# kubeflow/Code-Intelligence

Hardware: AMD Instinct MI355X
Metric: LM tokens/sec (whole node) (higher is better)
Workload: dtype bf16; 1 GPU; model=AWD-LSTM 4x2400 emb800 vocab60000, global_batch=512, seq_len=512, parallelism=dp1, device=MI355X

## Files before the change

### code_intelligence_amd/ops/crossentropy.py

```python
from __future__ import annotations

import os

import torch
from torch import Tensor

from . import extension as ext

__all__ = ["tied_decoder_ce", "TiedDecoderCE"]

_EMPTY = {}


def _empty_f32(device) -> Tensor:
    key = str(device)
    if key not in _EMPTY:
        _EMPTY[key] = torch.empty(0, dtype=torch.float32, device=device)
    return _EMPTY[key]


def _fp8r_enabled() -> bool:
    return os.environ.get("CI_CE_FP8R", "1") == "1"


_STORE = 448.0

_ONEPASS_MAX_V = 256 * 32 * 8

_ce_side = None


def _ce_side_stream():
    global _ce_side
    if _ce_side is None:
        _ce_side = torch.cuda.Stream()
    return _ce_side


def _ce_overlap_enabled() -> bool:
    return os.environ.get("CI_CE_2STREAM", "0") == "1"


class _FusedCEFp8Function(torch.autograd.Function):

    @staticmethod
    def forward(ctx, h: Tensor, weight: Tensor, bias: Tensor, targets: Tensor):
        lib = ext.require()
        f8 = torch.float8_e4m3fn
        N, H = h.shape
        V = weight.shape[0]
        C = int(os.environ.get("CI_CE_CHUNK", _FusedCEFunction.CHUNK))
        dev = h.device
        lse = torch.empty(N, dtype=torch.float32, device=dev)
        tgt_logit = torch.empty(N, dtype=torch.float32, device=dev)
        b32 = bias.to(torch.float32) if bias is not None else _empty_f32(dev)
        tgt64 = targets.to(torch.int64)
        sa = (h.detach().abs().amax().float() / 448.0).clamp_min(1e-12)
        sw = (weight.detach().abs().amax().float() / 448.0).clamp_min(1e-12)
        h8 = torch.empty(h.shape, dtype=f8, device=dev)
        lib.quantize_e4m3(h.detach().contiguous(), h8, sa)
        w8 = torch.empty(weight.shape, dtype=f8, device=dev)
        lib.quantize_e4m3(weight.detach().contiguous(), w8, sw)
        w8_t = w8.t()
        w_t = weight.t()
        logits_full = None
        if os.environ.get("CI_CE_SAVE_LOGITS", "1") != "0":
            try:
                logits_full = torch.empty(N, V, dtype=h.dtype, device=dev)
            except torch.cuda.OutOfMemoryError:
                pass
        dlog8_full = None
        if logits_full is not None and V <= _ONEPASS_MAX_V \
                and H % 16 == 0 and V % 16 == 0 \
                and N % 16 == 0 and min(C, N) % 16 == 0:
            try:
                dlog8_full = torch.empty(N, V, dtype=f8, device=dev)
            except torch.cuda.OutOfMemoryError:
                pass
        onepass = dlog8_full is not None
        if onepass:
            inv_n = (torch.ones((), dtype=torch.float32, device=dev)
                     / N).reshape(1)
        scratch = None if logits_full is not None else \
            torch.empty(min(C, N), V, dtype=h.dtype, device=dev)
        for s in range(0, N, C):
            e = min(N, s + C)
            logits = logits_full[s:e] if logits_full is not None \
                else scratch[: e - s]
            if (e - s) % 16 == 0 and H % 16 == 0 and V % 16 == 0:
                torch._scaled_mm(h8[s:e], w8_t, scale_a=sa, scale_b=sw,
                                 out_dtype=h.dtype, out=logits)
            else:
                torch.mm(h[s:e], w_t, out=logits)
            if onepass:
                lib.ce_onepass_dual(logits, tgt64[s:e], b32, lse[s:e],
                                    inv_n, dlog8_full[s:e], _STORE)
            else:
                lib.ce_rowstats(logits, tgt64[s:e], b32, lse[s:e],
                                tgt_logit[s:e])
        wrows = weight.detach()[tgt64]
        tgt_logit = (h.detach() * wrows).sum(dim=1, dtype=torch.float32)
        if bias is not None:
            tgt_logit = tgt_logit + b32[tgt64]
        loss = (lse - tgt_logit).mean()
        ctx.save_for_backward(h, weight, b32, tgt64, lse, w8, sw)
        ctx.logits_full = logits_full
        ctx.dlog8_full = dlog8_full
        ctx.h8 = h8 if logits_full is None else None
        ctx.sa = sa
        ctx.chunk = C
        ctx.has_bias = bias is not None
        ctx.bias_dtype = bias.dtype if bias is not None else None
        return loss

    @staticmethod
    def backward(ctx, dloss: Tensor):
        lib = ext.require()
        f8 = torch.float8_e4m3fn
        h, weight, b32, targets, lse, w8, sw = ctx.saved_tensors
        logits_full = ctx.logits_full
        ctx.logits_full = None
        h8, sa = ctx.h8, ctx.sa
        ctx.h8 = None
        dlog8_full = ctx.dlog8_full
        ctx.dlog8_full = None
        onepass = dlog8_full is not None
        has_bias = ctx.has_bias
        N, H = h.shape
        V = weight.shape[0]
        C = ctx.chunk
        dev = h.device
        dh = torch.empty_like(h)
        scale = (dloss / N).to(torch.float32).reshape(1)
        sc_over_store = (scale.reshape(()) / _STORE)
        scratch8 = None if onepass else \
            torch.empty(min(C, N), V, dtype=f8, device=dev)
        Haug = H + 16 if has_bias else H
        h_aug = h
        if has_bias:
            h_aug = torch.zeros(N, Haug, dtype=h.dtype, device=dev)
            h_aug[:, :H] = h
            h_aug[:, H] = 1
        dw_aug = torch.zeros(V, Haug, dtype=torch.float32, device=dev)
        recompute = None if logits_full is not None else \
            torch.empty(min(C, N), V, dtype=h.dtype, device=dev)
        w8_cm = w8.t().contiguous().t()
        w8_t = w8.t()
        w_t = weight.t()
        bias_arg = b32 if has_bias else _empty_f32(dev)
        overlap = _ce_overlap_enabled() and logits_full is not None
        side = _ce_side_stream() if overlap else None
        main = torch.cuda.current_stream() if overlap else None
        for s in range(0, N, C):
            e = min(N, s + C)
            c = e - s
            fp8_chunk = c % 16 == 0 and H % 16 == 0 and V % 16 == 0
            if logits_full is not None:
                dlog = logits_full[s:e]
            else:
                dlog = recompute[:c]
                if fp8_chunk:
                    torch._scaled_mm(h8[s:e], w8_t, scale_a=sa, scale_b=sw,
                                     out_dtype=h.dtype, out=dlog)
                else:
                    torch.mm(h[s:e], w_t, out=dlog)
            if onepass:
                dlog8 = dlog8_full[s:e]
            else:
                lib.ce_dlogits_dual(dlog, targets[s:e], bias_arg, lse[s:e],
                                    scale, scratch8, _STORE)
                dlog8 = scratch8[:c]
            if fp8_chunk:
                torch._scaled_mm(dlog8, w8_cm, scale_a=sc_over_store,
                                 scale_b=sw, out_dtype=h.dtype, out=dh[s:e])
            else:
                torch.mm(dlog, weight, out=dh[s:e])
            if overlap:
                side.wait_stream(main)
                with torch.cuda.stream(side):
                    dw_aug += torch.mm(dlog.t(), h_aug[s:e])
            else:
                dw_aug += torch.mm(dlog.t(), h_aug[s:e])
        if overlap:
            main.wait_stream(side)
        dw = dw_aug[:, :H]
        db = dw_aug[:, H] if has_bias else None
        if onepass:
            dl = dloss.to(torch.float32)
            dw_out = torch.empty(V, H, dtype=weight.dtype, device=dev)
            torch.mul(dw, dl, out=dw_out)
            return (dh, dw_out,
                    (db * dl).to(ctx.bias_dtype) if has_bias else None, None)
        return (dh, dw.to(weight.dtype),
                db.to(ctx.bias_dtype) if has_bias else None, None)


class _FusedCEFunction(torch.autograd.Function):
    CHUNK = int(os.environ.get("CI_CE_CHUNK", "65536"))

    @staticmethod
    def forward(ctx, h: Tensor, weight: Tensor, bias: Tensor, targets: Tensor):
        lib = ext.require()
        N, H = h.shape
        V = weight.shape[0]
        C = int(os.environ.get("CI_CE_CHUNK", _FusedCEFunction.CHUNK))
        lse = torch.empty(N, dtype=torch.float32, device=h.device)
        tgt_logit = torch.empty(N, dtype=torch.float32, device=h.device)
        b32 = bias.to(torch.float32) if bias is not None else _empty_f32(h.device)
        tgt64 = targets.to(torch.int64)
        save_logits = os.environ.get("CI_CE_SAVE_LOGITS", "1") != "0"
        logits_full = None
        if save_logits:
            try:
                logits_full = torch.empty(N, V, dtype=h.dtype, device=h.device)
            except torch.cuda.OutOfMemoryError:
                logits_full = None
        scratch = None if logits_full is not None else \
            torch.empty(min(C, N), V, dtype=h.dtype, device=h.device)
        w_t = weight.t()
        for s in range(0, N, C):
            e = min(N, s + C)
            logits = logits_full[s:e] if logits_full is not None \
                else scratch[: e - s]
            torch.mm(h[s:e], w_t, out=logits)
            lib.ce_rowstats(logits, tgt64[s:e], b32, lse[s:e], tgt_logit[s:e])
        loss = (lse - tgt_logit).mean()
        ctx.save_for_backward(h, weight, b32, tgt64, lse)
        ctx.logits_full = logits_full
        ctx.chunk = C
        ctx.has_bias = bias is not None
        ctx.bias_dtype = bias.dtype if bias is not None else None
        return loss

    @staticmethod
    def backward(ctx, dloss: Tensor):
        lib = ext.require()
        h, weight, b32, targets, lse = ctx.saved_tensors
        logits_full = ctx.logits_full
        ctx.logits_full = None
        has_bias = ctx.has_bias
        N, H = h.shape
        V = weight.shape[0]
        C = ctx.chunk
        dh = torch.empty_like(h)
        scale = (dloss / N).to(torch.float32).reshape(1)
        scratch = None if logits_full is not None else \
            torch.empty(min(C, N), V, dtype=h.dtype, device=h.device)
        w_t = weight.t()
        bias_arg = b32 if has_bias else _empty_f32(h.device)
        Haug = H + 16 if has_bias else H
        h_aug = h
        if has_bias:
            h_aug = torch.zeros(N, Haug, dtype=h.dtype, device=h.device)
            h_aug[:, :H] = h
            h_aug[:, H] = 1
        dw_aug = torch.zeros(V, Haug, dtype=torch.float32, device=h.device)
        for s in range(0, N, C):
            e = min(N, s + C)
            if logits_full is not None:
                dlog = logits_full[s:e]
            else:
                dlog = scratch[: e - s]
                torch.mm(h[s:e], w_t, out=dlog)
            lib.ce_dlogits(dlog, targets[s:e], bias_arg, lse[s:e], scale)
            torch.mm(dlog, weight, out=dh[s:e])
            dw_aug += torch.mm(dlog.t(), h_aug[s:e])
        dw = dw_aug[:, :H]
        db = dw_aug[:, H] if has_bias else None
        return (dh, dw.to(weight.dtype),
                db.to(ctx.bias_dtype) if has_bias else None, None)


@torch.no_grad()
def tied_decoder_accuracy(h: Tensor, weight: Tensor, bias: Tensor | None,
                          targets: Tensor, chunk: int = 16384) -> Tensor:
    h2 = h.reshape(-1, h.shape[-1])
    t2 = targets.reshape(-1)
    w_t = weight.t()
    correct = torch.zeros((), dtype=torch.long, device=h.device)
    for s in range(0, h2.shape[0], chunk):
        e = min(h2.shape[0], s + chunk)
        logits = torch.mm(h2[s:e], w_t)
        if bias is not None:
            logits += bias
        correct += (logits.argmax(dim=1) == t2[s:e]).sum()
    return correct.float() / max(1, h2.shape[0])


def tied_decoder_ce(h: Tensor, weight: Tensor, bias: Tensor | None,
                    targets: Tensor) -> Tensor:
    if h.is_cuda:
        if _fp8r_enabled() and h.dtype == torch.bfloat16 \
                and torch.is_grad_enabled() and h.requires_grad:
            return _FusedCEFp8Function.apply(h, weight, bias, targets)
        return _FusedCEFunction.apply(h, weight, bias, targets)
    logits = torch.nn.functional.linear(h.float(), weight.float(),
                                        bias.float() if bias is not None else None)
    return torch.nn.functional.cross_entropy(logits, targets)


class TiedDecoderCE(torch.nn.Module):

    def __init__(self, decoder: torch.nn.Linear):
        super().__init__()
        self.decoder = decoder

    def forward(self, h: Tensor, targets: Tensor) -> Tensor:
        return tied_decoder_ce(h.reshape(-1, h.shape[-1]), self.decoder.weight,
                               self.decoder.bias, targets.reshape(-1))
```

### code_intelligence_amd/ops/csrc/bindings.cpp

```cpp
#include <torch/extension.h>
#include <string>
#include <vector>

namespace ci {
void lstm_seq_forward_lib(at::Tensor xp, at::Tensor bias, at::Tensor h0,
                          at::Tensor c0, at::Tensor w_hh, at::Tensor hs,
                          at::Tensor cs, at::Tensor gates);
void lstm_seq_forward_fused(at::Tensor xp, at::Tensor bias, at::Tensor h0,
                            at::Tensor c0, at::Tensor w_hh, at::Tensor hs,
                            at::Tensor cs, at::Tensor gates);
void lstm_seq_forward_lib_fp8(at::Tensor xp, at::Tensor bias, at::Tensor h0,
                              at::Tensor c0, at::Tensor w8, at::Tensor wscale,
                              at::Tensor hs, at::Tensor cs, at::Tensor gates);
void quantize_e4m3(at::Tensor src, at::Tensor dst, at::Tensor scale);
void lstm_seq_forward_gemv(at::Tensor xp, at::Tensor bias, at::Tensor h0,
                           at::Tensor c0, at::Tensor w_hh, at::Tensor hs,
                           at::Tensor cs, at::Tensor gates);
long lstm_seq_forward_gemv_persistent(at::Tensor xp, at::Tensor bias,
                                      at::Tensor h0, at::Tensor c0,
                                      at::Tensor w_hh, at::Tensor hs,
                                      at::Tensor cs, at::Tensor gates,
                                      at::Tensor ws);
void lstm_seq_forward_gemv_fp8(at::Tensor xp, at::Tensor bias, at::Tensor h0,
                               at::Tensor c0, at::Tensor w8, at::Tensor wscale,
                               at::Tensor hs, at::Tensor cs, at::Tensor gates);
void lstm_seq_backward(at::Tensor dhs, at::Tensor dhT, at::Tensor dcT,
                       at::Tensor gates, at::Tensor hs, at::Tensor cs,
                       at::Tensor c0, at::Tensor w_hh, at::Tensor dgates,
                       at::Tensor dh0, at::Tensor dc0, bool need_dh0);
at::Tensor concat_pool(at::Tensor hidden, at::Tensor lengths);
std::vector<at::Tensor> concat_pool_fwd_idx(at::Tensor hidden,
                                            at::Tensor lengths, long max_len);
at::Tensor concat_pool_bwd(at::Tensor dout, at::Tensor argmax,
                           at::Tensor lengths, long max_len,
                           at::Tensor like_hidden);
std::vector<at::Tensor> qrnn_fo_pool_fwd(at::Tensor gates, at::Tensor c0);
std::vector<at::Tensor> qrnn_fo_pool_bwd(at::Tensor gates, at::Tensor c,
                                         at::Tensor c0, at::Tensor dh,
                                         at::Tensor dcT);
void ce_rowstats(at::Tensor logits, at::Tensor targets, at::Tensor bias,
                 at::Tensor lse, at::Tensor tgt);
void ce_dlogits(at::Tensor logits, at::Tensor targets, at::Tensor bias,
                at::Tensor lse, at::Tensor scale);
void ce_dlogits_dual(at::Tensor logits, at::Tensor targets, at::Tensor bias,
                     at::Tensor lse, at::Tensor scale, at::Tensor scratch8,
                     double store_scale);
void ce_onepass_dual(at::Tensor logits, at::Tensor targets, at::Tensor bias,
                     at::Tensor lse, at::Tensor scale, at::Tensor out8,
                     double store_scale);
at::Tensor artar_forward(at::Tensor out, at::Tensor r);
std::vector<at::Tensor> artar_backward(at::Tensor out, at::Tensor r,
                                       at::Tensor dloss, double ca, double cb);
void fused_adamw(std::vector<at::Tensor> params, std::vector<at::Tensor> grads,
                 std::vector<at::Tensor> masters, std::vector<at::Tensor> eas_,
                 std::vector<at::Tensor> eass, double lr, double b1, double b2,
                 double eps, double wd, double bc1, double bc2);
at::Tensor emb_gather(at::Tensor weight, at::Tensor ids, at::Tensor rowmask);
std::vector<std::string> tokenize_core(const std::string& text);
std::vector<std::vector<std::string>> tokenize_core_batch(
    const std::vector<std::string>& texts);
at::Tensor emb_scatter(at::Tensor gout, at::Tensor ids, at::Tensor rowmask,
                       long V, long pad_idx);
at::Tensor dropconnect_apply(at::Tensor w, long seed, double p);
void dropconnect_grad_(at::Tensor g, long seed, double p);
}

PYBIND11_MODULE(TORCH_EXTENSION_NAME, m) {
  m.def("lstm_seq_forward_lib", &ci::lstm_seq_forward_lib,
        "LSTM sequence forward (hipBLASLt GEMM + pointwise cell kernel)");
  m.def("lstm_seq_forward_fused", &ci::lstm_seq_forward_fused,
        "LSTM sequence forward (fused MFMA cell kernel)");
  m.def("lstm_seq_forward_lib_fp8", &ci::lstm_seq_forward_lib_fp8,
        "LSTM sequence forward (fp8 recurrent scaled_mm + pointwise cell)");
  m.def("quantize_e4m3", &ci::quantize_e4m3,
        "one-pass e4m3 quantize: dst = e4m3(src/scale)");
  m.def("lstm_seq_forward_gemv", &ci::lstm_seq_forward_gemv,
        "LSTM sequence forward (fused GEMV+cell kernel, small batch)");
  m.def("lstm_seq_forward_gemv_persistent",
        &ci::lstm_seq_forward_gemv_persistent,
        "whole-sequence persistent GEMV+cell kernel (grid barrier)");
  m.def("lstm_seq_forward_gemv_fp8", &ci::lstm_seq_forward_gemv_fp8,
        "LSTM sequence forward (fp8-weight GEMV+cell kernel)");
  m.def("lstm_seq_backward", &ci::lstm_seq_backward,
        "LSTM sequence backward (pointwise + per-step GEMM)",
        py::arg("dhs"), py::arg("dhT"), py::arg("dcT"), py::arg("gates"),
        py::arg("hs"), py::arg("cs"), py::arg("c0"), py::arg("w_hh"),
        py::arg("dgates"), py::arg("dh0"), py::arg("dc0"),
        py::arg("need_dh0") = true);
  m.def("concat_pool", &ci::concat_pool, "masked mean/max/last concat pool");
  m.def("concat_pool_fwd_idx", &ci::concat_pool_fwd_idx,
        "windowed strided concat pool -> (out, argmax); max_len <= 0: no window");
  m.def("concat_pool_bwd", &ci::concat_pool_bwd,
        "concat pool backward: dhidden laid out like like_hidden");
  m.def("qrnn_fo_pool_fwd", &ci::qrnn_fo_pool_fwd,
        "QRNN fo-pool forward scan (activates gates in place)");
  m.def("qrnn_fo_pool_bwd", &ci::qrnn_fo_pool_bwd,
        "QRNN fo-pool backward scan (pre-activation gate grads)");
  m.def("ce_rowstats", &ci::ce_rowstats, "CE row logsumexp + target logit");
  m.def("ce_dlogits", &ci::ce_dlogits, "in-place (softmax-onehot)*scale");
  m.def("ce_dlogits_dual", &ci::ce_dlogits_dual,
        "in-place bf16 dlogits + e4m3 scratch copy for the fp8 dh GEMM");
  m.def("ce_onepass_dual", &ci::ce_onepass_dual,
        "one read of the row: lse + in-place bf16 dlogits + e4m3 copy");
  m.def("artar_forward", &ci::artar_forward,
        "fused AR/TAR partial sums (one pass over out and r)");
  m.def("artar_backward", &ci::artar_backward,
        "fused AR/TAR gradient kernel (dout and dr in one pass)");
  m.def("fused_adamw", &ci::fused_adamw, "fused AdamW step");
  m.def("emb_gather", &ci::emb_gather, "embedding gather with row dropout");
  m.def("tokenize_core", &ci::tokenize_core, "native ASCII tokenizer core");
  m.def("tokenize_core_batch", &ci::tokenize_core_batch,
        "native ASCII tokenizer core (batch, GIL released)");
  m.def("emb_scatter", &ci::emb_scatter, "embedding grad scatter-add");
  m.def("dropconnect_apply", &ci::dropconnect_apply,
        "seeded DropConnect mask-scale (no mask tensor)");
  m.def("dropconnect_grad_", &ci::dropconnect_grad_,
        "in-place seeded DropConnect grad mask");
}
```

### code_intelligence_amd/ops/extension.py

```python
from __future__ import annotations

import importlib.util
import os
import sys
from pathlib import Path

import torch

_OPS_DIR = Path(__file__).resolve().parent
_CSRC = _OPS_DIR / "csrc"
_EXT_NAME = "_ci_hip"

_ext = None
_tried = False

SOURCES = [
    "bindings.cpp",
    "lstm_pointwise.hip",
    "lstm_gemm.hip",
    "lstm_gemv.hip",
    "pool.hip",
    "qrnn_pool.hip",
    "adam.hip",
    "ce.hip",
    "embedding.hip",
    "dropconnect.hip",
    "artar.hip",
    "fp8util.hip",
    "tokenizer.cpp",
]


def _find_so() -> Path | None:
    for cand in sorted(_OPS_DIR.glob(f"{_EXT_NAME}*.so")):
        return cand
    return None


def _warn_if_stale(so: Path) -> None:
    try:
        so_m = so.stat().st_mtime
        newer = [f.name for f in _CSRC.iterdir()
                 if f.suffix in (".hip", ".cpp", ".h")
                 and not f.name.endswith("_hip.hip")
                 and f.stat().st_mtime > so_m]
        if newer:
            import warnings
            warnings.warn(
                f"_ci_hip.so is older than kernel sources {newer}; "
                "rebuild with python -m code_intelligence_amd.ops.build",
                RuntimeWarning, stacklevel=3)
    except OSError:
        pass


def load(required: bool = False):
    global _ext, _tried
    if _ext is not None:
        return _ext
    if _tried and not required:
        return None
    _tried = True
    so = _find_so()
    if so is not None:
        _warn_if_stale(so)
    if so is None:
        if required:
            raise RuntimeError(
                "code_intelligence_amd HIP extension (_ci_hip*.so) not built. "
                "Run `python -m code_intelligence_amd.ops.build` (or "
                "__graft_entry__.build()). GPU ops refuse to run without the "
                "native gfx950 kernels — no silent eager fallback.")
        return None
    spec = importlib.util.spec_from_file_location(_EXT_NAME, so)
    mod = importlib.util.module_from_spec(spec)
    spec.loader.exec_module(mod)
    _ext = mod
    sys.modules[_EXT_NAME] = mod
    return _ext


def have() -> bool:
    return load(required=False) is not None


def require():
    return load(required=True)


def on_gpu(*tensors: torch.Tensor) -> bool:
    return any(t.is_cuda for t in tensors if isinstance(t, torch.Tensor))


def build(verbose: bool = True) -> Path:
    os.environ.setdefault("PYTORCH_ROCM_ARCH", "gfx950")
    from torch.utils.cpp_extension import load as jit_load

    build_dir = _OPS_DIR / "_build"
    build_dir.mkdir(exist_ok=True)
    for stale in _CSRC.glob("*_hip.hip"):
        stale.unlink()
    for stale in _CSRC.glob("*.prehip"):
        stale.unlink()
    sources = [str(_CSRC / s) for s in SOURCES if (_CSRC / s).exists()]
    mod = jit_load(
        name=_EXT_NAME,
        sources=sources,
        extra_cflags=["-O3", "-std=c++17"],
        extra_cuda_cflags=["-O3", "-std=c++17", "--offload-arch=gfx950"],
        build_directory=str(build_dir),
        verbose=verbose,
        is_python_module=True,
    )
    built = Path(mod.__file__)
    dest = _OPS_DIR / built.name
    if built.resolve() != dest.resolve():
        import shutil

        shutil.copy2(built, dest)
    global _ext
    _ext = mod
    return dest
```

### code_intelligence_amd/ops/lstm.py

```python
from __future__ import annotations

import os
from typing import Tuple

import torch
from torch import Tensor

from . import extension as ext

__all__ = ["lstm_forward", "sync_dw_stream"]

_side_stream = None


def _side() -> "torch.cuda.Stream":
    global _side_stream
    if _side_stream is None:
        _side_stream = torch.cuda.Stream()
    return _side_stream


def _side_dw_enabled() -> bool:
    return os.environ.get("CI_SIDE_DW", "0") == "1"


def sync_dw_stream() -> None:
    if _side_stream is not None and torch.cuda.is_available():
        torch.cuda.current_stream().wait_stream(_side_stream)


def _accum_grad(p: Tensor, g: Tensor) -> None:
    if p.grad is None:
        p.grad = g.detach().to(p.dtype)
    else:
        p.grad.add_(g.to(p.dtype))


def _fp8_weights(w_hh: Tensor):
    hit = getattr(w_hh, "_ci_fp8", None)
    if hit is not None and hit[0] == w_hh._version:
        return hit[1], hit[2]
    scale = w_hh.detach().abs().amax(dim=1, keepdim=True).float()         .clamp_min(1e-12) / 448.0
    q = (w_hh.detach().float() / scale).clamp(-448.0, 448.0)         .to(torch.float8_e4m3fn).view(torch.uint8).contiguous()
    out = (w_hh._version, q, scale.squeeze(1).contiguous())
    w_hh._ci_fp8 = out
    return out[1], out[2]


def _lstm_fp8_mode() -> str:
    return os.environ.get("CI_LSTM_FP8", "0")


def _lstm_fp8_enabled() -> bool:
    return _lstm_fp8_mode() in ("1", "all")


def _q8(lib, t: Tensor):
    scale = (t.detach().abs().amax().float() / 448.0).clamp_min(1e-12)
    q = torch.empty(t.shape, dtype=torch.float8_e4m3fn, device=t.device)
    lib.quantize_e4m3(t.detach().contiguous(), q, scale)
    return q, scale


def _cpu_lstm_loop(x: Tensor, h0: Tensor, c0: Tensor, w_ih: Tensor, w_hh: Tensor,
                   b_ih: Tensor, b_hh: Tensor) -> Tuple[Tensor, Tensor, Tensor]:
    B, T, _ = x.shape
    H = w_hh.shape[1]
    xp = torch.addmm((b_ih + b_hh), x.reshape(B * T, -1), w_ih.t()).view(B, T, 4 * H)
    h, c = h0, c0
    outs = []
    for t in range(T):
        gates = xp[:, t] + h @ w_hh.t()
        i, f, g, o = gates.chunk(4, dim=1)
        i, f, g, o = i.sigmoid(), f.sigmoid(), g.tanh(), o.sigmoid()
        c = f * c + i * g
        h = o * torch.tanh(c)
        outs.append(h)
    return torch.stack(outs, dim=1), h, c


class _FusedLSTMFunction(torch.autograd.Function):

    @staticmethod
    def forward(ctx, x, h0, c0, w_ih, w_hh, b_ih, b_hh):
        lib = ext.require()
        B, T, In = x.shape
        H = w_hh.shape[1]
        dt = x.dtype
        x_tm = x.transpose(0, 1).contiguous()
        bias = (b_ih + b_hh).to(torch.float32)
        h0 = h0.contiguous()
        c32 = c0.to(torch.float32).contiguous()
        shapes_ok = (dt == torch.bfloat16 and B > 8 and B % 16 == 0
                     and (T * B) % 16 == 0 and In % 16 == 0 and H % 16 == 0)
        fp8 = _lstm_fp8_enabled() and shapes_ok
        fp8_xp = fp8 or (_lstm_fp8_mode() == "xp" and shapes_ok)
        if fp8_xp:
            x2 = x_tm.view(T * B, In)
            x8, sx = _q8(lib, x2)
            wih8, swi = _q8(lib, w_ih)
            xp = torch._scaled_mm(x8, wih8.t(), scale_a=sx, scale_b=swi,
                                  out_dtype=dt).view(T, B, 4 * H)
        else:
            xp = torch.mm(x_tm.view(T * B, In), w_ih.t()).view(T, B, 4 * H)
        hs = torch.empty(T, B, H, dtype=dt, device=x.device)
        cs = torch.empty(T, B, H, dtype=torch.float32, device=x.device)
        gates = torch.empty(T, B, 4 * H, dtype=dt, device=x.device)
        mode = os.environ.get("CI_LSTM_MODE", "lib")
        if dt == torch.bfloat16 and B <= 8 and mode != "lib-only":
            if os.environ.get("CI_SERVE_FP8W", "0") == "1"                     and not torch.is_grad_enabled():
                w8, wscale = _fp8_weights(w_hh)
                lib.lstm_seq_forward_gemv_fp8(xp, bias, h0, c32, w8,
                                              wscale, hs, cs, gates)
            elif os.environ.get("CI_SERVE_PERSISTENT", "0") == "1" \
                    and not getattr(_FusedLSTMFunction, "_pers_failed", False):
                ws = torch.zeros(4, dtype=torch.int32, device=x.device)
                nb = lib.lstm_seq_forward_gemv_persistent(
                    xp, bias, h0, c32, w_hh, hs, cs, gates, ws)
                if nb == 0 or int(ws[2].item()) != 0:
                    import warnings
                    warnings.warn("persistent GEMV unavailable "
                                  f"(nb={nb}); per-step fallback (sticky)")
                    _FusedLSTMFunction._pers_failed = True
                    lib.lstm_seq_forward_gemv(xp, bias, h0, c32,
                                              w_hh, hs, cs, gates)
            else:
                lib.lstm_seq_forward_gemv(xp, bias, h0, c32,
                                          w_hh, hs, cs, gates)
        elif dt == torch.bfloat16 and H % 8 == 0 and (
                mode == "fused"
                or (mode == "auto" and H >= 2048 and B >= 128)):
            lib.lstm_seq_forward_fused(xp, bias, h0, c32, w_hh,
                                       hs, cs, gates)
        elif fp8 and mode == "lib":
            whh8, swh = _q8(lib, w_hh)
            lib.lstm_seq_forward_lib_fp8(xp, bias, h0, c32, whh8, swh,
                                         hs, cs, gates)
        else:
            lib.lstm_seq_forward_lib(xp, bias, h0, c32, w_hh,
                                     hs, cs, gates)
        ctx.save_for_backward(x_tm, h0, c0, w_ih, w_hh, gates, hs, cs)
        ctx.direct_params = (w_ih, b_ih, b_hh)
        hT = hs[-1].clone()
        cT = cs[-1].to(dt)
        out = hs.transpose(0, 1)
        return out, hT, cT

    @staticmethod
    def backward(ctx, dhs, dhT, dcT):
        lib = ext.require()
        x_tm, h0, c0, w_ih, w_hh, gates, hs, cs = ctx.saved_tensors
        T, B, In = x_tm.shape
        H = w_hh.shape[1]
        dt = x_tm.dtype
        dhs_tm = dhs.transpose(0, 1).contiguous()
        dgates = torch.empty(T, B, 4 * H, dtype=dt, device=x_tm.device)
        dh0 = torch.empty(B, H, dtype=torch.float32, device=x_tm.device)
        need_dh0 = ctx.needs_input_grad[1]
        dc0 = torch.empty(B, H, dtype=torch.float32, device=x_tm.device)
        lib.lstm_seq_backward(dhs_tm, dhT.contiguous(),
                              dcT.to(torch.float32).contiguous(),
                              gates, hs, cs,
                              c0.to(torch.float32).contiguous(), w_hh,
                              dgates, dh0, dc0, need_dh0)
        dh0_out = dh0.to(dt) if need_dh0 else None
        dg2 = dgates.view(T * B, 4 * H)
        dx_tm = torch.mm(dg2, w_ih).view(T, B, In)
        dw_hh = torch.mm(dgates[0].t(), h0.to(dt))
        if T > 1:
            dw_hh += torch.mm(dgates[1:].reshape((T - 1) * B, 4 * H).t(),
                              hs[:-1].reshape((T - 1) * B, H))
        if _side_dw_enabled() and ctx.needs_input_grad[3]:
            pw, pbi, pbh = ctx.direct_params
            s_ = _side()
            s_.wait_stream(torch.cuda.current_stream())
            dg2.record_stream(s_)
            x_tm.record_stream(s_)
            with torch.cuda.stream(s_):
                dw_ih_s = torch.mm(dg2.t(), x_tm.view(T * B, In))
                db_s = dg2.sum(dim=0)
                _accum_grad(pw, dw_ih_s)
                _accum_grad(pbi, db_s)
                _accum_grad(pbh, db_s.clone())
            return (dx_tm.transpose(0, 1), dh0_out, dc0.to(dt),
                    None, dw_hh.to(w_hh.dtype), None, None)
        dw_ih = torch.mm(dg2.t(), x_tm.view(T * B, In))
        db = dg2.sum(dim=0).to(dt)
        return (dx_tm.transpose(0, 1), dh0_out, dc0.to(dt),
                dw_ih.to(w_ih.dtype), dw_hh.to(w_hh.dtype), db, db.clone())


def lstm_forward(x: Tensor, h0: Tensor, c0: Tensor, w_ih: Tensor, w_hh: Tensor,
                 b_ih: Tensor, b_hh: Tensor):
    if x.is_cuda:
        hs, hT, cT = _FusedLSTMFunction.apply(x, h0, c0, w_ih, w_hh, b_ih, b_hh)
        return hs, (hT, cT)
    out, h, c = _cpu_lstm_loop(x, h0, c0, w_ih, w_hh, b_ih, b_hh)
    return out, (h, c)
```

Before: 630,300 tokens/s.

## Compute weight gradients as K-major NN GEMMs via tiled LDS transpose pack

Adds a HIP tiled-transpose kernel (pack_kmajor) that packs activations into K-major layout so the weight-gradient GEMMs become NN GEMMs producing transposed results, which are transposed back afterwards. The LSTM backward now fuses dW_ih and dW_hh into one GEMM over a packed [x ; h_prev] operand when the heuristic allows. The tied-decoder CE backward likewise accumulates dW^T from a pre-transposed, bias-augmented h. This targets the cost of TN GEMMs with a strided reduction dimension, and it adds extra transpose passes and temporary buffers.

```diff
diff --git a/code_intelligence_amd/ops/crossentropy.py b/code_intelligence_amd/ops/crossentropy.py
--- a/code_intelligence_amd/ops/crossentropy.py
+++ b/code_intelligence_amd/ops/crossentropy.py
@@ -39,6 +39,24 @@
 
 def _ce_overlap_enabled() -> bool:
     return os.environ.get("CI_CE_2STREAM", "0") == "1"
+
+
+def _h_aug_t(lib, h: Tensor, has_bias: bool) -> Tensor:
+    N, H = h.shape
+    Haug = H + 16 if has_bias else H
+    h_augT = torch.empty(Haug, N, dtype=h.dtype, device=h.device)
+    lib.pack_kmajor(h.detach().contiguous(), h_augT, 0, 0)
+    if has_bias:
+        h_augT[H] = 1
+        h_augT[H + 1:] = 0
+    return h_augT
+
+
+def _split_dw_aug_t(lib, dw_augT: Tensor, H: int, has_bias: bool):
+    dw = torch.empty(dw_augT.shape[1], H, dtype=dw_augT.dtype,
+                     device=dw_augT.device)
+    lib.pack_kmajor(dw_augT[:H], dw, 0, 0)
+    return dw, (dw_augT[H] if has_bias else None)
 
 
 class _FusedCEFp8Function(torch.autograd.Function):
@@ -135,13 +153,9 @@
         sc_over_store = (scale.reshape(()) / _STORE)
         scratch8 = None if onepass else \
             torch.empty(min(C, N), V, dtype=f8, device=dev)
-        Haug = H + 16 if has_bias else H
-        h_aug = h
-        if has_bias:
-            h_aug = torch.zeros(N, Haug, dtype=h.dtype, device=dev)
-            h_aug[:, :H] = h
-            h_aug[:, H] = 1
-        dw_aug = torch.zeros(V, Haug, dtype=torch.float32, device=dev)
+        h_augT = _h_aug_t(lib, h, has_bias)
+        dw_augT = torch.zeros(h_augT.shape[0], V, dtype=torch.float32,
+                              device=dev)
         recompute = None if logits_full is not None else \
             torch.empty(min(C, N), V, dtype=h.dtype, device=dev)
         w8_cm = w8.t().contiguous().t()
@@ -178,13 +192,12 @@
             if overlap:
                 side.wait_stream(main)
                 with torch.cuda.stream(side):
-                    dw_aug += torch.mm(dlog.t(), h_aug[s:e])
-            else:
-                dw_aug += torch.mm(dlog.t(), h_aug[s:e])
+                    dw_augT += torch.mm(h_augT[:, s:e], dlog)
+            else:
+                dw_augT += torch.mm(h_augT[:, s:e], dlog)
         if overlap:
             main.wait_stream(side)
-        dw = dw_aug[:, :H]
-        db = dw_aug[:, H] if has_bias else None
+        dw, db = _split_dw_aug_t(lib, dw_augT, H, has_bias)
         if onepass:
             dl = dloss.to(torch.float32)
             dw_out = torch.empty(V, H, dtype=weight.dtype, device=dev)
@@ -248,13 +261,9 @@
             torch.empty(min(C, N), V, dtype=h.dtype, device=h.device)
         w_t = weight.t()
         bias_arg = b32 if has_bias else _empty_f32(h.device)
-        Haug = H + 16 if has_bias else H
-        h_aug = h
-        if has_bias:
-            h_aug = torch.zeros(N, Haug, dtype=h.dtype, device=h.device)
-            h_aug[:, :H] = h
-            h_aug[:, H] = 1
-        dw_aug = torch.zeros(V, Haug, dtype=torch.float32, device=h.device)
+        h_augT = _h_aug_t(lib, h, has_bias)
+        dw_augT = torch.zeros(h_augT.shape[0], V, dtype=torch.float32,
+                              device=h.device)
         for s in range(0, N, C):
             e = min(N, s + C)
             if logits_full is not None:
@@ -264,9 +273,8 @@
                 torch.mm(h[s:e], w_t, out=dlog)
             lib.ce_dlogits(dlog, targets[s:e], bias_arg, lse[s:e], scale)
             torch.mm(dlog, weight, out=dh[s:e])
-            dw_aug += torch.mm(dlog.t(), h_aug[s:e])
-        dw = dw_aug[:, :H]
-        db = dw_aug[:, H] if has_bias else None
+            dw_augT += torch.mm(h_augT[:, s:e], dlog)
+        dw, db = _split_dw_aug_t(lib, dw_augT, H, has_bias)
         return (dh, dw.to(weight.dtype),
                 db.to(ctx.bias_dtype) if has_bias else None, None)
 
diff --git a/code_intelligence_amd/ops/csrc/bindings.cpp b/code_intelligence_amd/ops/csrc/bindings.cpp
--- a/code_intelligence_amd/ops/csrc/bindings.cpp
+++ b/code_intelligence_amd/ops/csrc/bindings.cpp
@@ -1,5 +1,6 @@
 #include <torch/extension.h>
 #include <string>
+#include <tuple>
 #include <vector>
 
 namespace ci {
@@ -63,6 +64,10 @@
                        long V, long pad_idx);
 at::Tensor dropconnect_apply(at::Tensor w, long seed, double p);
 void dropconnect_grad_(at::Tensor g, long seed, double p);
+void pack_kmajor(at::Tensor src, at::Tensor dst, long row_off, long col_off);
+std::tuple<at::Tensor, at::Tensor> lstm_weight_grads(
+    at::Tensor dgates, at::Tensor x_tm, at::Tensor hs, at::Tensor h0,
+    bool need_ih, bool need_hh);
 }
 
 PYBIND11_MODULE(TORCH_EXTENSION_NAME, m) {
@@ -116,4 +121,12 @@
         "seeded DropConnect mask-scale (no mask tensor)");
   m.def("dropconnect_grad_", &ci::dropconnect_grad_,
         "in-place seeded DropConnect grad mask");
+  m.def("pack_kmajor", &ci::pack_kmajor,
+        "dst[row_off + c, col_off + r] = src[r, c] (tiled LDS transpose)",
+        py::arg("src"), py::arg("dst"), py::arg("row_off") = 0,
+        py::arg("col_off") = 0);
+  m.def("lstm_weight_grads", &ci::lstm_weight_grads,
+        "LSTM dW_ih/dW_hh: K-major pack of [x ; h_prev] + one NN GEMM",
+        py::arg("dgates"), py::arg("x_tm"), py::arg("hs"), py::arg("h0"),
+        py::arg("need_ih") = true, py::arg("need_hh") = true);
 }
diff --git a/code_intelligence_amd/ops/csrc/kmajor_pack.hip b/code_intelligence_amd/ops/csrc/kmajor_pack.hip
--- /dev/null
+++ b/code_intelligence_amd/ops/csrc/kmajor_pack.hip
@@ -0,0 +1,145 @@
+#include "common.h"
+
+#include <cstdint>
+#include <tuple>
+
+namespace ci {
+
+template <typename U, bool VLD, bool VST>
+__global__ __launch_bounds__(256) void pack_kmajor_kernel(
+    const U* __restrict__ src, U* __restrict__ dst, long R, long C,
+    long ld_dst, long row_off, long col_off) {
+  constexpr int VEC = 16 / sizeof(U);
+  constexpr int TILE = 16 * VEC;
+  __shared__ __attribute__((aligned(16))) U tile[TILE * TILE];
+  const long r0 = (long)blockIdx.x * TILE;
+  const long c0 = (long)blockIdx.y * TILE;
+  const int l16 = threadIdx.x & 15;
+  const int grp = threadIdx.x >> 4;
+
+  #pragma unroll
+  for (int i = 0; i < TILE / 16; ++i) {
+    const int rl = grp + 16 * i;
+    const long r = r0 + rl, c = c0 + l16 * VEC;
+    __attribute__((aligned(16))) U v[VEC];
+    if (VLD && r < R && c + VEC <= C) {
+      *reinterpret_cast<int4*>(v) =
+          *reinterpret_cast<const int4*>(src + r * C + c);
+    } else {
+      #pragma unroll
+      for (int e = 0; e < VEC; ++e)
+        v[e] = (r < R && c + e < C) ? src[r * C + c + e] : U(0);
+    }
+    const int slot = l16 ^ ((rl / VEC) & 15);
+    *reinterpret_cast<int4*>(&tile[rl * TILE + slot * VEC]) =
+        *reinterpret_cast<const int4*>(v);
+  }
+  __syncthreads();
+
+  #pragma unroll
+  for (int i = 0; i < TILE / 16; ++i) {
+    const int cl = grp + 16 * i;
+    const long c = c0 + cl;
+    if (c >= C) continue;
+    const int slot = (cl / VEC) ^ l16;
+    __attribute__((aligned(16))) U v[VEC];
+    #pragma unroll
+    for (int e = 0; e < VEC; ++e)
+      v[e] = tile[(l16 * VEC + e) * TILE + slot * VEC + (cl % VEC)];
+    const long r = r0 + l16 * VEC;
+    U* p = dst + (row_off + c) * ld_dst + col_off + r;
+    if (VST && r + VEC <= R) {
+      *reinterpret_cast<int4*>(p) = *reinterpret_cast<const int4*>(v);
+    } else {
+      #pragma unroll
+      for (int e = 0; e < VEC; ++e)
+        if (r + e < R) p[e] = v[e];
+    }
+  }
+}
+
+template <typename U>
+static void launch_pack(const at::Tensor& src, at::Tensor& dst, long R, long C,
+                        long row_off, long col_off) {
+  constexpr int VEC = 16 / sizeof(U);
+  constexpr int TILE = 16 * VEC;
+  const long ld = dst.size(1);
+  const U* s = reinterpret_cast<const U*>(src.data_ptr());
+  U* d = reinterpret_cast<U*>(dst.data_ptr());
+  const bool vld = C % VEC == 0 && reinterpret_cast<uintptr_t>(s) % 16 == 0;
+  const bool vst = ld % VEC == 0 && col_off % VEC == 0 &&
+                   reinterpret_cast<uintptr_t>(d) % 16 == 0;
+  const dim3 grid(ceil_div(R, TILE), ceil_div(C, TILE));
+  TORCH_CHECK(grid.y <= 65535, "pack_kmajor: too many columns");
+#define CI_PACK_LAUNCH(VLD, VST)                                            \
+  hipLaunchKernelGGL((pack_kmajor_kernel<U, VLD, VST>), grid, dim3(256), 0, \
+                     stream(), s, d, R, C, ld, row_off, col_off)
+  if (vld && vst) CI_PACK_LAUNCH(true, true);
+  else if (vld) CI_PACK_LAUNCH(true, false);
+  else if (vst) CI_PACK_LAUNCH(false, true);
+  else CI_PACK_LAUNCH(false, false);
+#undef CI_PACK_LAUNCH
+}
+
+void pack_kmajor(at::Tensor src, at::Tensor dst, long row_off, long col_off) {
+  CI_CHECK_CUDA(src); CI_CHECK_CUDA(dst);
+  CI_CHECK_CONTIG(src); CI_CHECK_CONTIG(dst);
+  TORCH_CHECK(src.dim() == 2 && dst.dim() == 2, "pack_kmajor: 2-D tensors");
+  TORCH_CHECK(src.scalar_type() == dst.scalar_type(),
+              "pack_kmajor: src/dst dtype mismatch");
+  const long R = src.size(0), C = src.size(1);
+  TORCH_CHECK(row_off >= 0 && col_off >= 0 && row_off + C <= dst.size(0) &&
+              col_off + R <= dst.size(1),
+              "pack_kmajor: target block outside dst");
+  if (R == 0 || C == 0) return;
+  switch (src.scalar_type()) {
+    case at::ScalarType::BFloat16:
+    case at::ScalarType::Half:
+      launch_pack<uint16_t>(src, dst, R, C, row_off, col_off); break;
+    case at::ScalarType::Float:
+      launch_pack<uint32_t>(src, dst, R, C, row_off, col_off); break;
+    default:
+      TORCH_CHECK(false, "pack_kmajor: unsupported dtype ", src.scalar_type());
+  }
+}
+
+std::tuple<at::Tensor, at::Tensor> lstm_weight_grads(
+    at::Tensor dgates, at::Tensor x_tm, at::Tensor hs, at::Tensor h0,
+    bool need_ih, bool need_hh) {
+  CI_CHECK_CUDA(dgates); CI_CHECK_CONTIG(dgates); CI_CHECK_CONTIG(x_tm);
+  CI_CHECK_CONTIG(hs); CI_CHECK_CONTIG(h0);
+  TORCH_CHECK(dgates.dim() == 3 && x_tm.dim() == 3 && hs.dim() == 3 &&
+              h0.dim() == 2, "lstm_weight_grads: bad ranks");
+  const long T = dgates.size(0), B = dgates.size(1), G = dgates.size(2);
+  const long In = x_tm.size(2), H = hs.size(2);
+  TORCH_CHECK(G == 4 * H && x_tm.size(0) == T && x_tm.size(1) == B &&
+              hs.size(0) == T && hs.size(1) == B && h0.size(0) == B &&
+              h0.size(1) == H, "lstm_weight_grads: shape mismatch");
+  const auto dt = dgates.scalar_type();
+  TORCH_CHECK(x_tm.scalar_type() == dt && hs.scalar_type() == dt &&
+              h0.scalar_type() == dt, "lstm_weight_grads: dtype mismatch");
+  at::Tensor dw_ih, dw_hh;
+  if (!need_ih && !need_hh) return {dw_ih, dw_hh};
+  const long rows_ih = need_ih ? In : 0;
+  const long rows = rows_ih + (need_hh ? H : 0);
+  at::Tensor packed = at::empty({rows, T * B}, dgates.options());
+  if (need_ih) pack_kmajor(x_tm.view({T * B, In}), packed, 0, 0);
+  if (need_hh) {
+    pack_kmajor(h0, packed, rows_ih, 0);
+    if (T > 1)
+      pack_kmajor(hs.narrow(0, 0, T - 1).view({(T - 1) * B, H}), packed,
+                  rows_ih, B);
+  }
+  at::Tensor dwT = at::mm(packed, dgates.view({T * B, G}));
+  if (need_ih) {
+    dw_ih = at::empty({G, In}, dgates.options());
+    pack_kmajor(dwT.narrow(0, 0, In), dw_ih, 0, 0);
+  }
+  if (need_hh) {
+    dw_hh = at::empty({G, H}, dgates.options());
+    pack_kmajor(dwT.narrow(0, rows_ih, H), dw_hh, 0, 0);
+  }
+  return {dw_ih, dw_hh};
+}
+
+}
diff --git a/code_intelligence_amd/ops/extension.py b/code_intelligence_amd/ops/extension.py
--- a/code_intelligence_amd/ops/extension.py
+++ b/code_intelligence_amd/ops/extension.py
@@ -27,6 +27,7 @@
     "dropconnect.hip",
     "artar.hip",
     "fp8util.hip",
+    "kmajor_pack.hip",
     "tokenizer.cpp",
 ]
 
diff --git a/code_intelligence_amd/ops/lstm.py b/code_intelligence_amd/ops/lstm.py
--- a/code_intelligence_amd/ops/lstm.py
+++ b/code_intelligence_amd/ops/lstm.py
@@ -60,6 +60,28 @@
     q = torch.empty(t.shape, dtype=torch.float8_e4m3fn, device=t.device)
     lib.quantize_e4m3(t.detach().contiguous(), q, scale)
     return q, scale
+
+
+def _kmajor_dw(T: int, B: int, In: int, H: int, dt) -> bool:
+    if os.environ.get("CI_LSTM_DW", "") == "legacy":
+        return False
+    if dt not in (torch.bfloat16, torch.float32):
+        return False
+    if T * B < _KMAJOR_MIN_K:
+        return True
+    return (In + H) * 4 * H >= 256 * 256 * _n_cus()
+
+
+_KMAJOR_MIN_K = 4096
+_cus = None
+
+
+def _n_cus() -> int:
+    global _cus
+    if _cus is None:
+        _cus = torch.cuda.get_device_properties(
+            torch.cuda.current_device()).multi_processor_count
+    return _cus
 
 
 def _cpu_lstm_loop(x: Tensor, h0: Tensor, c0: Tensor, w_ih: Tensor, w_hh: Tensor,
@@ -166,11 +188,18 @@
         dh0_out = dh0.to(dt) if need_dh0 else None
         dg2 = dgates.view(T * B, 4 * H)
         dx_tm = torch.mm(dg2, w_ih).view(T, B, In)
-        dw_hh = torch.mm(dgates[0].t(), h0.to(dt))
-        if T > 1:
-            dw_hh += torch.mm(dgates[1:].reshape((T - 1) * B, 4 * H).t(),
-                              hs[:-1].reshape((T - 1) * B, H))
-        if _side_dw_enabled() and ctx.needs_input_grad[3]:
+        need_ih, need_hh = ctx.needs_input_grad[3], ctx.needs_input_grad[4]
+        side = _side_dw_enabled() and need_ih
+        if side or not _kmajor_dw(T, B, In, H, dt):
+            dw_hh = torch.mm(dgates[0].t(), h0.to(dt))
+            if T > 1:
+                dw_hh += torch.mm(dgates[1:].reshape((T - 1) * B, 4 * H).t(),
+                                  hs[:-1].reshape((T - 1) * B, H))
+            dw_ih = None
+        else:
+            dw_ih, dw_hh = lib.lstm_weight_grads(dgates, x_tm, hs, h0.to(dt),
+                                                 need_ih, need_hh)
+        if side:
             pw, pbi, pbh = ctx.direct_params
             s_ = _side()
             s_.wait_stream(torch.cuda.current_stream())
@@ -184,10 +213,13 @@
                 _accum_grad(pbh, db_s.clone())
             return (dx_tm.transpose(0, 1), dh0_out, dc0.to(dt),
                     None, dw_hh.to(w_hh.dtype), None, None)
-        dw_ih = torch.mm(dg2.t(), x_tm.view(T * B, In))
+        if dw_ih is None and need_ih:
+            dw_ih = torch.mm(dg2.t(), x_tm.view(T * B, In))
         db = dg2.sum(dim=0).to(dt)
         return (dx_tm.transpose(0, 1), dh0_out, dc0.to(dt),
-                dw_ih.to(w_ih.dtype), dw_hh.to(w_hh.dtype), db, db.clone())
+                dw_ih.to(w_ih.dtype) if dw_ih is not None else None,
+                dw_hh.to(w_hh.dtype) if dw_hh is not None else None,
+                db, db.clone())
 
 
 def lstm_forward(x: Tensor, h0: Tensor, c0: Tensor, w_ih: Tensor, w_hh: Tensor,
```

New measurement: 665,600 tokens/s (median of 6 runs). +5.6%, better.
